# nannau/DoWnGAN

Measured on AMD Instinct MI355X. Metric: train-step samples/sec (G+D+GP), higher is better.
Workload: dtype bf16

## Files before the change

### downgan_amd/_lib.py

```python
from __future__ import annotations

import ctypes as C
import os

_HERE = os.path.dirname(os.path.abspath(__file__))
LIB_PATH = os.environ.get("DG_LIB_OVERRIDE") or os.path.join(_HERE, "csrc", "libdowngan_hip.so")

DG_F32, DG_BF16 = 0, 1
STATUS = {0: "DG_OK", -1: "DG_ERR_BAD_SHAPE", -2: "DG_ERR_BAD_DTYPE", -3: "DG_ERR_BAD_ARG", -4: "DG_ERR_LAUNCH"}


class Epilogue(C.Structure):
    _fields_ = [("bias", C.c_void_p), ("has_act", C.c_int), ("act_slope", C.c_float),
                ("r1", C.c_void_p), ("ldr1", C.c_int64), ("s1", C.c_float),
                ("r2", C.c_void_p), ("ldr2", C.c_int64), ("s2", C.c_float),
                ("mask", C.c_void_p), ("ldmask", C.c_int64), ("mask_slope", C.c_float),
                ("accumulate", C.c_int), ("mask_bits", C.c_void_p), ("out_bits", C.c_void_p),
                ("mask_c0", C.c_int), ("mask_last", C.c_int), ("out_q", C.c_void_p), ("out_qs", C.c_void_p), ("ldqs", C.c_int64),
                ("out_u", C.c_void_p), ("out_ue", C.c_void_p), ("skip_y", C.c_int), ("out_amax", C.c_void_p)]


class ConvGeom(C.Structure):
    _fields_ = [("dtype", C.c_int), ("N", C.c_int), ("H", C.c_int), ("W", C.c_int),
                ("Cin", C.c_int), ("Cout", C.c_int), ("stride", C.c_int), ("cin_real", C.c_int), ("pixel_shuffle", C.c_int),
# ... 110 lines not shown

class TemporalSpec(C.Structure):
    _fields_ = [("speed_u", C.c_int), ("speed_v", C.c_int), ("nthr", C.c_int), ("ndur", C.c_int), ("nlag", C.c_int),
                ("nbins", C.c_int), ("below", C.c_int * TEMPORAL_MAX_THR), ("lag", C.c_int * TEMPORAL_MAX_LAGS),
                ("scale", C.c_float * EOF_MAX_C), ("offset", C.c_float * EOF_MAX_C),
                ("thr", (C.c_float * TEMPORAL_MAX_THR) * HIST_MAX_OUT), ("lo", (C.c_float * TEMPORAL_MAX_LAGS) * HIST_MAX_OUT),
                ("inv_w", (C.c_float * TEMPORAL_MAX_LAGS) * HIST_MAX_OUT)]


MINMAX_PARTS = 256
_vp, _i, _i64, _f = C.c_void_p, C.c_int, C.c_int64, C.c_float
_PROTOS = {
    "dg_conv3x3_fwd": [C.POINTER(ConvGeom), C.POINTER(Epilogue), _vp, _vp, _vp, _vp],
    "dg_conv3x3_dgrad": [C.POINTER(ConvGeom), C.POINTER(Epilogue), _vp, _vp, _vp, _vp],
    "dg_conv3x3_wgrad": [C.POINTER(ConvGeom), _vp, _vp, _vp, _vp, _vp],
    "dg_conv3x3_wgrad_dense": [_vp, _i, _vp, _vp, _vp, _vp, _vp],
    "dg_conv3x3_wgrad_f8": [C.POINTER(ConvGeom), _vp, _vp, _vp, _vp, _vp, _vp],
    "dg_exp_from_amax": [_vp, _i, _i, _vp, _vp],
    "dg_conv3x3_wgrad_dense_f8": [C.POINTER(ConvGeom), _i, _vp, _vp, _vp, _vp, _vp, _vp],
    "dg_gather_gemm": [C.POINTER(GGDesc), C.POINTER(Epilogue), _vp, _vp, _vp, _vp],
    "dg_conv3x3_plan": [C.POINTER(ConvGeom), _i, C.POINTER(GGDesc)],
    "dg_last_conv_kernels": [],
    "dg_last_wgrad_kernel": [],
    "dg_conv3x3_dgrad_launches": [C.POINTER(ConvGeom)],
    "dg_conv3x3_dgrad_stream_eligible": [C.POINTER(ConvGeom), C.POINTER(Epilogue)],
    "dg_set_s2_dgrad_stream": [C.c_int],
    "dg_colsum": [_i, _vp, _i64, _i64, _i64, _i64, _i, _vp, _vp],
    "dg_colsum_multi": [_i, _vp, _i64, _i64, _i, _i, _vp, _vp],
    "dg_repack_conv_weights": [_i, _i, _vp, _vp, _i, _i, _vp],
    "dg_repack_dense_dgrad": [_i, _vp, _i, _i, _vp, _vp],
    "dg_wgrad_unswap": [_vp, _vp, _i, _i, _vp],
    "dg_linear_fwd": [_i, _vp, _i64, _vp, _i64, _vp, _i, _i, _i, _i64, _vp],
    "dg_linear_dx": [_i, _i, _vp, _i, _vp, _i64, _vp, _i64, _vp, _i64, _f, _i, _i, _i64, _vp],
    "dg_linear_dw": [_i, _vp, _i, _vp, _i64, _vp, _i64, _i, _i, _i64, _vp],
    "dg_linear_dw_wide": [_i, _vp, _i, _vp, _i64, _vp, _i64, _i, _i, _i64, _i, _vp],
    "dg_bias_act": [_i, _vp, _i, _vp, _vp, _i, _i, _i, _i, _f, _vp, _i, _f, _vp],
    "dg_mask_mul": [_i, _vp, _i64, _vp, _i64, _i64, _i, _f, _vp],
    "dg_axpby": [_i, _vp, _i64, _vp, _i64, _f, _vp, _i64, _f, _i64, _i, _vp],
    "dg_gp_interp": [_i, _vp, _vp, _vp, _vp, _i, _i64, _vp],
    "dg_gp_interp_c2": [_i, _vp, _vp, _i64, _vp, _vp, _vp, _vp, _i, _i64, _vp],
    "dg_scale_rows_c2": [_i, _vp, _i64, _vp, _vp, _i, _i64, _vp],
    "dg_sumsq_rows": [_i, _vp, _i, _i64, _vp, _vp],
    "dg_gp_finish": [_vp, _i, _i, _f, _f, _vp, _vp, _vp],
    "dg_scale_rows": [_i, _vp, _vp, _vp, _i, _i64, _vp],
    "dg_l1": [_i, _vp, _i64, _vp, _i64, _i64, _i, _vp, _vp, _i64, _f, _vp, _i64, _vp],
    "dg_sqdiff": [_i, _vp, _i64, _vp, _i64, _i64, _i, _vp, _vp],
    "dg_sum_strided": [_vp, _i, _i, _f, _vp, _vp],
    "dg_fill_col": [_vp, _i, _i, _i, _f, _vp],
    "dg_adam": [_vp, _vp, _vp, _vp, _vp, _i64, _f, _f, _f, _f, _i, _f, _vp],
    "dg_nchw_to_nhwc": [_i, _vp, _vp, _i, _i, _i, _i, _i, _vp],
    "dg_nhwc_to_nchw": [_i, _vp, _i64, _vp, _i, _i, _i, _i, _vp],
    "dg_cast": [_i, _vp, _vp, _i64, _vp],
    "dg_minmax_partial": [_i, _vp, _i64, _i64, _i, _vp, _vp],
    "dg_minmax_finish": [_vp, _i, _vp, _vp],
    "dg_normalise_planar": [_i, _vp, _i, _i, _i, _i64, _i, _vp, _vp, _vp],
    "dg_ssim_level": [_vp, _vp, _i, _i, _i, C.POINTER(SsimParams), _vp, _vp],
    "dg_avgpool2": [_vp, _vp, _i, _i, _i, _vp],
    "dg_msssim_finish": [_vp, _i, _i, C.POINTER(MsssimCombine), _vp, _vp],
    "dg_div_vort_sums": [_i, _vp, _i64, _vp, _i64, _i, _i, _i, _vp, _vp],
    "dg_gather_samples": [_i, _vp, _i64, _i, _vp, _i, _vp, _i, _vp],
    "dg_quant_mxfp8": [_i, _vp, _i64, _i64, _i, _vp, _i64, _vp, _i64, _vp],
    "dg_block_exp_max": [_vp, _i64, _i64, _i, _i, _vp, _vp, _vp],
    "dg_block_exp_max_batch": [C.POINTER(ExpBatch), _i, _vp, _vp],
    "dg_quant_uniform": [_i, _vp, _i64, _i64, _i, _vp, _vp, _i64, _vp],
    "dg_conv3x3_fwd_f8": [C.POINTER(ConvGeom), C.POINTER(Epilogue), C.POINTER(F8Operands), _vp, _vp],
    "dg_conv3x3_dgrad_f8": [C.POINTER(ConvGeom), C.POINTER(Epilogue), C.POINTER(F8Operands), _vp, _vp],
# ... 120 lines not shown
```

### downgan_amd/csrc/elementwise.hip

```cpp
#include <cstdlib>
#include "dg_internal.h"
#include <type_traits>

#include <math.h>

static inline unsigned ew_blocks(long long nthreads) {
  long long b = (nthreads + 255) / 256;
  if (b > 256 * 16) b = 256 * 16;
  if (b < 1) b = 1;
  return (unsigned)b;
}

template <typename T> __device__ __forceinline__ void ldc(const T* p, float* v) {
  ld4(p, v);
  if constexpr (DT<T>::EPC == 8) ld4(p + 4, v + 4);
}
template <typename T> __device__ __forceinline__ void stc(T* p, const float* v) {
  st4(p, v);
  if constexpr (DT<T>::EPC == 8) st4(p + 4, v + 4);
}

template <typename T>
__global__ void mask_mul_kernel(T* u, long long ldu, const T* y, long long ldy, long long rows, int cchunks, float slope) {
  constexpr int EPC = DT<T>::EPC;
// ... 394 lines not shown
}
extern "C" int dg_bias_act(int out_dtype, const float* in, int ldi, const float* bias, void* out, int ldo, int rows, int C,
                           int has_act, float slope, const void* mask, int ldmask, float mask_slope, void* stream) {
  if (!in || !out || rows <= 0 || C <= 0) return DG_ERR_BAD_SHAPE;
  hipStream_t st = reinterpret_cast<hipStream_t>(stream);
  const unsigned nb = ew_blocks((long long)rows * C);
  if (out_dtype == DG_F32) hipLaunchKernelGGL(bias_act_kernel<float>, dim3(nb), dim3(256), 0, st, in, ldi, bias, (float*)out, ldo, rows, C, has_act, slope, (const float*)mask, ldmask, mask_slope);
  else if (out_dtype == DG_BF16) hipLaunchKernelGGL(bias_act_kernel<bf16_t>, dim3(nb), dim3(256), 0, st, in, ldi, bias, (bf16_t*)out, ldo, rows, C, has_act, slope, (const bf16_t*)mask, ldmask, mask_slope);
  else return DG_ERR_BAD_DTYPE;
  return dg_check_launch();
}

__global__ void sum_strided_kernel(const float* in, int n, int stride, float scale, float* out) {
  float s = 0.f;
  for (int i = threadIdx.x; i < n; i += 64) s += in[(long long)i * stride];
  s = wave_sum(s);
  if (threadIdx.x == 0) out[0] = s * scale;
}
extern "C" int dg_sum_strided(const float* in, int n, int stride, float scale, float* out, void* stream) {
  if (!in || !out || n <= 0) return DG_ERR_BAD_ARG;
  hipLaunchKernelGGL(sum_strided_kernel, dim3(1), dim3(64), 0, reinterpret_cast<hipStream_t>(stream), in, n, stride, scale, out);
  return dg_check_launch();
}

__global__ void fill_col_kernel(float* buf, int rows, int ld, int col, float value) {
  for (int r = blockIdx.x * blockDim.x + threadIdx.x; r < rows; r += gridDim.x * blockDim.x) buf[(long long)r * ld + col] = value;
}
extern "C" int dg_fill_col(float* buf, int rows, int ld, int col, float value, void* stream) {
  if (!buf || rows <= 0) return DG_ERR_BAD_ARG;
  hipLaunchKernelGGL(fill_col_kernel, dim3(ew_blocks(rows)), dim3(256), 0, reinterpret_cast<hipStream_t>(stream), buf, rows, ld, col, value);
  return dg_check_launch();
}

__global__ void adam_kernel(float* p, const float* g, float* m, float* v, bf16_t* shadow, long long n4, float step_size,
                            float beta1, float beta2, float eps, float inv_sqrt_bc2, float gscale) {
  for (long long i = (long long)blockIdx.x * blockDim.x + threadIdx.x; i < n4; i += (long long)gridDim.x * blockDim.x) {
    float4 pv = reinterpret_cast<float4*>(p)[i];
    const float4 gv = reinterpret_cast<const float4*>(g)[i];
    float4 mv = reinterpret_cast<float4*>(m)[i];
    float4 vv = reinterpret_cast<float4*>(v)[i];
    float pa[4] = {pv.x, pv.y, pv.z, pv.w}, ga[4] = {gv.x, gv.y, gv.z, gv.w};
    float ma[4] = {mv.x, mv.y, mv.z, mv.w}, va[4] = {vv.x, vv.y, vv.z, vv.w};
#pragma unroll
    for (int e = 0; e < 4; ++e) {
      const float gg = ga[e] * gscale;
      ma[e] = beta1 * ma[e] + (1.f - beta1) * gg;
      va[e] = beta2 * va[e] + (1.f - beta2) * gg * gg;
      const float denom = sqrtf(va[e]) * inv_sqrt_bc2 + eps;
      pa[e] -= step_size * (ma[e] / denom);
    }
    reinterpret_cast<float4*>(p)[i] = make_float4(pa[0], pa[1], pa[2], pa[3]);
    reinterpret_cast<float4*>(m)[i] = make_float4(ma[0], ma[1], ma[2], ma[3]);
    reinterpret_cast<float4*>(v)[i] = make_float4(va[0], va[1], va[2], va[3]);
    if (shadow) st4(shadow + 4 * i, pa);
  }
}
extern "C" int dg_adam(float* p, const float* g, float* m, float* v, void* shadow_bf16, int64_t n, float lr, float beta1,
                       float beta2, float eps, int step, float grad_scale, void* stream) {
  if (!p || !g || !m || !v || n <= 0 || n % 4 || step < 1) return DG_ERR_BAD_ARG;
  const double bc1 = 1.0 - pow((double)beta1, step), bc2 = 1.0 - pow((double)beta2, step);
  hipLaunchKernelGGL(adam_kernel, dim3(ew_blocks(n / 4)), dim3(256), 0, reinterpret_cast<hipStream_t>(stream), p, g, m, v,
                     (bf16_t*)shadow_bf16, (long long)(n / 4), (float)(lr / bc1), beta1, beta2, eps, (float)(1.0 / sqrt(bc2)), grad_scale);
  return dg_check_launch();
}

template <typename T>
__global__ void nchw_to_nhwc_kernel(const float* src, T* dst, int N, int C, int H, int W, int Cpad) {
  const long long npix = (long long)N * H * W, hw = (long long)H * W;
  const long long total = npix * Cpad;
  for (long long i = (long long)blockIdx.x * blockDim.x + threadIdx.x; i < total; i += (long long)gridDim.x * blockDim.x) {
    const int c = (int)(i / npix); const long long pix = i % npix;
    const long long n = pix / hw, r = pix % hw;
    const float v = c < C ? src[(n * C + c) * hw + r] : 0.f;
    st_elem(dst + pix * Cpad + c, v);
  }
}
extern "C" int dg_nchw_to_nhwc(int dtype, const float* src, void* dst, int N, int C, int H, int W, int Cpad, void* stream) {
  if (!src || !dst || N <= 0 || C <= 0 || H <= 0 || W <= 0 || Cpad < C) return DG_ERR_BAD_SHAPE;
  hipStream_t st = reinterpret_cast<hipStream_t>(stream);
  const unsigned nb = ew_blocks((long long)N * H * W * Cpad);
  if (dtype == DG_F32) hipLaunchKernelGGL(nchw_to_nhwc_kernel<float>, dim3(nb), dim3(256), 0, st, src, (float*)dst, N, C, H, W, Cpad);
  else if (dtype == DG_BF16) hipLaunchKernelGGL(nchw_to_nhwc_kernel<bf16_t>, dim3(nb), dim3(256), 0, st, src, (bf16_t*)dst, N, C, H, W, Cpad);
  else return DG_ERR_BAD_DTYPE;
// ... 129 lines not shown
```

### downgan_amd/csrc/linear.hip

```cpp
#include "dg_internal.h"
#include <stdlib.h>

template <typename T> struct MmaL;
template <> struct MmaL<bf16_t> {
  static __device__ __forceinline__ void run(const uint4& a, const uint4& b, f32x4_t& c) {
    c = __builtin_amdgcn_mfma_f32_16x16x32_bf16(__builtin_bit_cast(bf16x8_t, a), __builtin_bit_cast(bf16x8_t, b), c, 0, 0, 0);
  }
};
template <> struct MmaL<float> {
  static __device__ __forceinline__ void run(const uint4& a, const uint4& b, f32x4_t& c) {
    c = __builtin_amdgcn_mfma_f32_16x16x4f32(__uint_as_float(a.x), __uint_as_float(b.x), c, 0, 0, 0);
    c = __builtin_amdgcn_mfma_f32_16x16x4f32(__uint_as_float(a.y), __uint_as_float(b.y), c, 0, 0, 0);
    c = __builtin_amdgcn_mfma_f32_16x16x4f32(__uint_as_float(a.z), __uint_as_float(b.z), c, 0, 0, 0);
    c = __builtin_amdgcn_mfma_f32_16x16x4f32(__uint_as_float(a.w), __uint_as_float(b.w), c, 0, 0, 0);
  }
};

typedef __attribute__((ext_vector_type(2))) float dg_f32x2_t;
template <typename T> struct LdX4;
typedef __attribute__((ext_vector_type(2))) unsigned int dg_u32x2_t;
template <> struct LdX4<float> {
  typedef dg_u32x4_t raw;
  static __device__ __forceinline__ raw load(const float* row, unsigned voff) {
    return __builtin_amdgcn_raw_buffer_load_b128(__builtin_amdgcn_make_buffer_rsrc((void*)row, 0, -1, 0x00020000), voff, 0, 0);
// ... 224 lines not shown
        acc[4 * q + e][0] = __builtin_elementwise_fma(d2, wa, acc[4 * q + e][0]);
        acc[4 * q + e][1] = __builtin_elementwise_fma(d2, wb, acc[4 * q + e][1]);
      }
  };
  auto wrow = [&](int o) { return LdX4<T>::load(w + (long long)(o < O ? o : O - 1) * ldw, voff); };
  constexpr int PD = 6;
  typename LdX4<T>::raw wq[PD];
#pragma unroll
  for (int u = 0; u < PD; ++u) wq[u] = wrow(u);
  read_row(d[0], 0);
  for (int o = 0; o < O; o += PD) {
#pragma unroll
    for (int u = 0; u < PD; ++u) {
      read_row(d[(u + 1) & 1], o + u + 1 < O ? o + u + 1 : O);
      landed(d[u & 1]);
      row_fma(wq[u], d[u & 1]);
      wq[u] = wrow(o + u + PD);
    }
  }
#pragma unroll
  for (int b = 0; b < BG; ++b) {
    if (b0 + b >= B) break;
    float v[4] = {acc[b][0][0], acc[b][0][1], acc[b][1][0], acc[b][1][1]};
    if (mask) {
      float mv[4];
      ld4(mask + (long long)(b0 + b) * ldmask + k, mv);
#pragma unroll
      for (int e = 0; e < 4; ++e) v[e] *= leaky_grad(mv[e], slope);
    }
    st4(dx + (long long)(b0 + b) * lddx + k, v);
  }
}

extern "C" int dg_linear_dx(int dtype, int out_dtype, const float* dy, int ldo, const void* w, int64_t ldw, void* dx,
                            int64_t lddx, const void* mask, int64_t ldmask, float mask_slope, int B, int O, int64_t K,
                            void* stream) {
  if (!dy || !w || !dx) return DG_ERR_BAD_ARG;
  if (B <= 0 || O <= 0 || O > 128 || K <= 0 || K % 8 || ldw % 8 || lddx % 8) return DG_ERR_BAD_SHAPE;
  if (mask && ldmask % 8) return DG_ERR_BAD_SHAPE;
  hipStream_t st = reinterpret_cast<hipStream_t>(stream);
  if (K >= 4096 && (long long)K * 4 < (1ll << 32) && B >= 16) {
    dim3 gridw((unsigned)((K / 4 + 255) / 256), (unsigned)((B + 31) / 32));
    if (dtype == DG_F32 && out_dtype == DG_F32) {
      hipLaunchKernelGGL((lin_dx_wide_kernel<float, float>), gridw, dim3(256), 0, st, dy, ldo, (const float*)w, (long long)ldw, (float*)dx,
                         (long long)lddx, (const float*)mask, (long long)ldmask, mask_slope, B, O, (long long)K);
      return dg_check_launch();
    }
    if (dtype == DG_BF16 && out_dtype == DG_BF16) {
      hipLaunchKernelGGL((lin_dx_wide_kernel<bf16_t, bf16_t>), gridw, dim3(256), 0, st, dy, ldo, (const bf16_t*)w, (long long)ldw, (bf16_t*)dx,
                         (long long)lddx, (const bf16_t*)mask, (long long)ldmask, mask_slope, B, O, (long long)K);
      return dg_check_launch();
    }
  }
  constexpr int BG = 16;
  const int epc = dtype == DG_F32 ? 4 : 8;
  dim3 grid((unsigned)((K / epc + 255) / 256), (unsigned)((B + BG - 1) / BG));
  if (dtype == DG_F32 && out_dtype == DG_F32)
    hipLaunchKernelGGL((lin_dx_kernel<float, float, BG>), grid, dim3(256), 0, st, dy, ldo, (const float*)w, ldw,
                       (float*)dx, lddx, (const float*)mask, ldmask, mask_slope, B, O, K);
  else if (dtype == DG_BF16 && out_dtype == DG_BF16)
    hipLaunchKernelGGL((lin_dx_kernel<bf16_t, bf16_t, BG>), grid, dim3(256), 0, st, dy, ldo, (const bf16_t*)w, ldw,
                       (bf16_t*)dx, lddx, (const bf16_t*)mask, ldmask, mask_slope, B, O, K);
  else if (dtype == DG_BF16 && out_dtype == DG_F32)
    hipLaunchKernelGGL((lin_dx_kernel<bf16_t, float, BG>), grid, dim3(256), 0, st, dy, ldo, (const bf16_t*)w, ldw,
                       (float*)dx, lddx, (const bf16_t*)mask, ldmask, mask_slope, B, O, K);
  else
    return DG_ERR_BAD_DTYPE;
  return dg_check_launch();
}

template <typename T, int OT>
__global__ __launch_bounds__(256) void lin_dw_kernel(const float* __restrict__ dy, int ldo, const T* __restrict__ x,
                                                     long long ldx, float* dw, long long lddw, int B, int O,
// ... 137 lines not shown
```

### downgan_amd/engine.py

```python
from __future__ import annotations

import dataclasses
import math
import os

import torch

from . import layout
from .ops import Conv

G_SLOPE = 0.01
C_SLOPE = 0.2
RES_SCALE = 0.2
FC_HID = 100
FC_HID_P = 112
FC_HID_LD = 128
FC_OUT_P = 16


@dataclasses.dataclass
class HyperParams:
    gp_lambda: float = 10.0
    critic_iterations: int = 5
    batch_size: int = 32
    gamma: float = 0.01
    content_lambda: float = 5.0
    lr: float = 0.00025
    beta1: float = 0.9
    beta2: float = 0.99
    eps: float = 1e-8


class ParamStore:

    def __init__(self, ops):
        self.ops = ops
        self.entries = {}
        self.size = 0
        self.conv_dgrad = {}
        self.after_refresh = []
        self._pending = None

    def add(self, name, shape):
        n = int(math.prod(shape))
        assert n % 4 == 0, (name, shape)
        self.entries[name] = (self.size, n, tuple(shape))
        self.size += n

    def finalize(self):
        o = self.ops
        self.p = o.zeros(self.size, dtype=torch.float32)
        self.g = o.zeros(self.size, dtype=torch.float32)
        self.m = o.zeros(self.size, dtype=torch.float32)
        self.v = o.zeros(self.size, dtype=torch.float32)
        self.shadow = self.p if o.tdtype == torch.float32 else o.zeros(self.size)
        self.dgrad_pack = {k: o.zeros(co * 9 * ci) for k, (co, ci) in self.conv_dgrad.items()}
        self.t = 0

    def defer(self, fn):
        self.sync()
        self._pending = fn

    def sync(self):
        fn, self._pending = self._pending, None
        if fn is not None:
            fn()

    def view(self, buf, name):
        if self._pending is not None:
            self.sync()
        off, n, shape = self.entries[name]
        return buf[off:off + n].view(shape)

    def master(self, name):
        return self.view(self.p, name)

    def grad(self, name):
        return self.view(self.g, name)

    def w(self, name):
        if self._pending is not None:
            self.sync()
        off, n, _ = self.entries[name]
        return self.shadow[off:off + n]

    def w2d(self, name):
        return self.view(self.shadow, name)

    def wd(self, name):
        if self._pending is not None:
            self.sync()
        return self.dgrad_pack[name]

    def refresh(self, shadow_done=False):
        o = self.ops
        if o.tdtype != torch.float32 and not shadow_done:
            o.cast(self.p, self.shadow)
        for name, (co, ci) in self.conv_dgrad.items():
            o.repack(self.master(name).reshape(-1), self.dgrad_pack[name], co, ci, 1)
        for fn in self.after_refresh:
            fn()

    def zero_grad(self, skip=None):
        self.sync()
        if skip is None:
            self.g.zero_()
        else:
            off, n, _ = self.entries[skip]
            self.g[:off].zero_()
            self.g[off + n:].zero_()

    def adam_step(self, hp: HyperParams, grad_scale=1.0):
        self.t += 1
        o = self.ops
        o.adam(self.p, self.g, self.m, self.v, None if o.tdtype == torch.float32 else self.shadow,
               hp.lr, hp.beta1, hp.beta2, hp.eps, self.t, grad_scale)
        self.refresh(shadow_done=True)

    def load_host(self, packed: dict):
        self.sync()
        host = torch.zeros(self.size, dtype=torch.float32)
        for name, t in packed.items():
            off, n, shape = self.entries[name]
            assert tuple(t.shape) == shape, (name, t.shape, shape)
            host[off:off + n] = t.reshape(-1)
        self.p.copy_(host)
        self.refresh()

    def export_state(self):
        self.sync()
        return self.p, self.m, self.v, self.t

    def import_state(self, state):
        p, m, v, t = state
        assert p.numel() == self.size, (p.numel(), self.size)
        self.sync()
        self.p.copy_(p); self.m.copy_(m); self.v.copy_(v)
        self.t = int(t)
        self.refresh()

    def to_host(self, buf=None):
        self.sync()
        h = (self.p if buf is None else buf).detach().cpu()
        return {name: h[off:off + n].view(shape).clone() for name, (off, n, shape) in self.entries.items()}


class NativeCritic:

    STRIDES = (1, 2, 1, 2, 1, 2, 1, 2)

    def __init__(self, ops, coarse_dim, fine_dim, nc, batch, stacked=False):
        assert fine_dim % 16 == 0, "critic.py:95 needs fine_dim divisible by 16"
        self.ops, self.B = ops, batch
        self.cd, self.fine, self.nc = coarse_dim, fine_dim, nc
        cd = coarse_dim
        self.c_real = [nc, cd, cd, 2 * cd, 2 * cd, 4 * cd, 4 * cd, 8 * cd, 8 * cd]
        self.c_pad = [layout.pad16(c) for c in self.c_real]
        self.convs = []
        h = fine_dim
        for l, st in enumerate(self.STRIDES):
            self.convs.append(Conv(batch, h, h, self.c_pad[l], self.c_pad[l + 1], st, False,
                                   cin_real=(nc if l == 0 and nc <= 2 else 0), net="C",
                                   cin_alg=self.c_real[l], cout_alg=self.c_real[l + 1]))
            h //= st
        self.hf = h
        self.fc_k = h * h * self.c_pad[8]
        P = self.P = ParamStore(ops)
        for l, cv in enumerate(self.convs):
            P.add(f"features.{2 * l}.weight", (cv.Cout, 9, cv.Cin))
            P.conv_dgrad[f"features.{2 * l}.weight"] = (cv.Cout, cv.Cin)
        P.add("features.0.bias", (self.c_pad[1],))
        P.add("classifier.0.weight", (FC_HID_P, self.fc_k))
        P.add("classifier.0.bias", (FC_HID_LD,))
        P.add("classifier.2.weight", (FC_OUT_P, FC_HID_LD))
        P.add("classifier.2.bias", (FC_OUT_P,))
        P.finalize()
        o = ops
        use_bits = os.environ.get("DG_NO_MASK_BITS") is None and all(c >= 128 and c % 64 == 0 for c in self.c_pad[1:])
        self.f8 = bool(getattr(o, "f8", False))
        self.stacked = bool(stacked) and use_bits and not self.f8 and 3 * batch <= 128 and os.environ.get("DG_NO_FC1_FUSED") is None
        self.stack_from = (int(stacked) - 1 if (stacked is not True and int(stacked) > 1) else 0) if self.stacked else 0
        cap = 3 * batch if self.stacked else batch
        self.cap = cap
        full = lambda cv: (cap,) + tuple(o.out_shape(cv))[1:]
        self._acts_all = [o.zeros(*full(cv)) for cv in self.convs[:7]] + [None]
        self._us_all = [o.zeros(*full(cv)) for cv in self.convs]
        self._bits_all = [o.zeros(*o.bits_shape(full(cv)), dtype=torch.int16) for cv in self.convs] if use_bits else None
        self.acts = [a[:batch] if a is not None else o.zeros(*o.out_shape(self.convs[7])) for a in self._acts_all]
        self.us = [u[:batch] for u in self._us_all]
        self.act_bits = [b[:batch] for b in self._bits_all] if use_bits else None
        self._h1pre_all = o.zeros(cap, FC_HID_LD, dtype=torch.float32)
        self._h1_all = o.zeros(cap, FC_HID_LD)
        self._outpre_all = o.zeros(cap, FC_OUT_P, dtype=torch.float32)
        self._out_all = o.zeros(cap, FC_OUT_P, dtype=torch.float32)
        self._dout_all = o.zeros(cap, FC_OUT_P, dtype=torch.float32)
        self.uh1 = o.zeros(batch, FC_HID_LD, dtype=torch.float32)
        self._cv_cache = {}
        self._tan = self._th1pre = self._th1 = self._ones = None
        self.fc1_fused = 3 * batch <= 128 and os.environ.get("DG_NO_FC1_FUSED") is None
        if self.fc1_fused:
            self._y7_all = o.zeros(4 * batch, *self.acts[7].shape[1:])
            self._uh1_all = o.zeros(3 * batch, FC_HID_LD, dtype=torch.float32)
            self.acts[7] = self._y7_all[3 * batch:]
            if self.stacked:
                self._acts_all[7] = self._y7_all[:3 * batch]
        qbuf = lambda t: (o.zeros(*t.shape, dtype=torch.uint8), o.zeros(*t.shape[:-1], t.shape[-1] // 32, dtype=torch.uint8))
        self.actq = [None] * 8
        self.usq = [None] * 8
        self.wq_f, self.wq_d = [None] * 8, [None] * 8
# ... 331 lines not shown
                for p in range(3):
                    r = slice(p * B, (p + 1) * B)
                    o.conv_dgrad(cv1[l], self._us_all[l][r], P.wd(name), self._us_all[l - 1][r], mask_bits=self._bits_all[l - 1][r], mask_slope=C_SLOPE)
            elif l > 0:
                o.conv_dgrad(cv3[l], self._us_all[l], P.wd(name), self._us_all[l - 1], mask_bits=self._bits_all[l - 1], mask_slope=C_SLOPE)
            else:
                o.conv_dgrad(cv1[0], self._us_all[0][2 * B:], P.wd(name), dx)


class NativeGenerator:

    def __init__(self, ops, filters, channels, batch, coarse_side, n_predictands=2, num_res_blocks=16, num_upsample=3):
        assert filters % 16 == 0, "native path needs filters to be a multiple of 16"
        self.ops, self.B, self.S = ops, batch, coarse_side
        self.F, self.cin, self.npred = filters, channels, n_predictands
        self.cin_p, self.np_p = layout.pad16(channels), layout.pad16(n_predictands)
        self.nrb, self.nup = num_res_blocks, num_upsample
        F_, S, B = filters, coarse_side, batch
        self.cv_conv1 = Conv(B, S, S, self.cin_p, F_, cin_real=(channels if channels <= 2 else 0), cin_alg=channels)
        self.cv_b = [Conv(B, S, S, k * F_, F_, net="G") for k in range(1, 6)]
        self.cv_conv2 = Conv(B, S, S, F_, F_, net="G")
        self.cv_up = [Conv(B, S << u, S << u, F_, 4 * F_, 1, True, net="T") for u in range(num_upsample)]
        hs = S << num_upsample
        self.cv_c30 = Conv(B, hs, hs, F_, F_, net="T")
        self.cv_c32 = Conv(B, hs, hs, F_, self.np_p, cout_alg=n_predictands)
        self.cv_c32_bwd = Conv(B, hs, hs, self.np_p, F_, cin_real=n_predictands, cin_alg=n_predictands) if n_predictands <= 2 else None
        P = self.P = ParamStore(ops)
        for name, cv, _, _, dgrad in self._conv_layers():
            P.add(name + ".weight", (cv.Cout, 9, cv.Cin))
            P.add(name + ".bias", (cv.Cout,))
            if dgrad:
                P.conv_dgrad[name + ".weight"] = (cv.Cout, cv.Cin)
        P.finalize()
        o = ops
        self.ndrb = 3 * num_res_blocks
        self.out1 = o.zeros(B, S, S, F_)
        self.trunk = o.zeros(B, S, S, F_)
        self.ups = [o.zeros(B, S << (u + 1), S << (u + 1), F_) for u in range(num_upsample)]
        self.c30 = o.zeros(B, hs, hs, F_)
        self.fake = o.zeros(B, hs, hs, self.np_p)
        self._ring = [o.zeros(B, S, S, 5 * F_) for _ in range(4)]
        self._saved = None
        self._bwd = None
        self.f8 = bool(getattr(o, "f8_generator", False)) and all(o.f8_eligible(cv, "fwd") for cv in self.cv_b)
        self._qring = [(o.zeros(B, S, S, 5 * F_, dtype=torch.uint8), o.zeros(B, S, S, 5 * F_ // 32, dtype=torch.uint8)) for _ in range(4)] if self.f8 else None
        self.f8_tail = self.f8 and all(o.f8_eligible(cv, "fwd") for cv in self.cv_up + [self.cv_c30])
        self._tq = None
        self._w_c32_bwd = o.zeros(F_ * 9 * self.np_p) if self.cv_c32_bwd is not None else None
        self._dw_c32_tmp = None
        if self.cv_c32_bwd is not None:
            P.after_refresh.append(lambda: o.repack(P.master("conv3.2.weight").reshape(-1), self._w_c32_bwd, self.np_p, F_, 2))
        self._wq = {}
        self._vq = None
        self._qlast = None
        self.cv_v = [Conv(B, S, S, F_, (5 - j) * F_, net="G") for j in range(5)]
        self._vsize = [(5 - j) * F_ * 9 * F_ for j in range(5)]
        self._vpack = [o.zeros(sum(self._vsize)) for _ in range(self.ndrb)]
        self.f8_bwd = self.f8 and bool(getattr(o, "f8_gbwd", False)) and all(o.f8_eligible(cv, "dgrad") for cv in self.cv_v)
        self.f8_wg = (self.f8_bwd and bool(getattr(o, "f8_wgrad", False)) and bool(getattr(o, "f8_gwgrad", False)) and F_ == 128 and S % 64 == 0)
        self._slab_u = self._us_u = self._ex = self._eu = self._ex_new = self._eu_new = None
        self._u_ok = False
        self._u_live = False
        P.after_refresh.append(self._rebuild_vpacks)
        if self.f8:
            P.after_refresh.append(self._requantise_weights)

# ... 562 lines not shown
```

### downgan_amd/ops.py

```python
from __future__ import annotations

import ctypes as C
import dataclasses

import os
import torch

from . import _lib
from ._lib import ConvGeom, Epilogue, check

TORCH_DTYPE = {"f32": torch.float32, "bf16": torch.bfloat16}
DG_DTYPE = {"f32": _lib.DG_F32, "bf16": _lib.DG_BF16}


@dataclasses.dataclass(frozen=True)
class Conv:
    N: int
    H: int
    W: int
    Cin: int
    Cout: int
    stride: int = 1
    pixel_shuffle: bool = False
    cin_real: int = 0
# ... 93 lines not shown
        assert 1 <= len(bufs) <= _lib.FINITE_MAX
        f = _lib.FiniteBufs(nbuf=len(bufs))
        for i, (name, t) in enumerate(bufs):
            assert t.is_cuda and t.is_contiguous() and t.dtype in (torch.float32, torch.bfloat16), (name, t.dtype)
            f.ptr[i], f.n[i], f.dtype[i] = t.data_ptr(), t.numel(), (_lib.DG_F32 if t.dtype == torch.float32 else _lib.DG_BF16)
        if self._finite_counts is None:
            self._finite_counts = torch.zeros(_lib.FINITE_MAX, dtype=torch.int32, device=self.device)
        check(self.lib.dg_count_nonfinite(C.byref(f), _ptr(self._finite_counts), self._stream()), "dg_count_nonfinite")
        counts = self._finite_counts.cpu().tolist()
        return {name: int(counts[i]) for i, (name, _) in enumerate(bufs)}

    def _stream(self):
        if torch.cuda.current_device() != self._dev_index:
            torch.cuda.set_device(self.device)
        return C.c_void_p(torch.cuda.current_stream(self.device).cuda_stream)

    per_layer = False

    def _timed(self, tag, flops, fn, nbytes=0.0, net="", geom=""):
        if self.prof is None:
            return fn()
        s, e = torch.cuda.Event(enable_timing=True), torch.cuda.Event(enable_timing=True)
        s.record()
        rc = fn()
        e.record()
        if self.per_layer and geom:
            tag = f"{tag}:{geom}"
        if net:
            tag = f"{tag}:{net}"
        if tag.startswith(("conv_fwd", "conv_dgrad")):
            tag = f"{tag}:k{self.lib.dg_last_conv_kernels()}"
        self.prof.append((tag, flops, nbytes, s, e))
        return rc

    @staticmethod
    def _geom_tag(cv):
        return f"{cv.Cin}>{cv.Cout}@{cv.H}" + ("s2" if cv.stride == 2 else "") + ("ps" if cv.pixel_shuffle else "")

    @staticmethod
    def conv_flops(cv):
        return 2.0 * 9 * (cv.cin_alg or cv.Cin) * (cv.cout_alg or cv.Cout) * cv.Ho * cv.Wo * cv.N

    def conv_bytes(self, cv, ep=None):
        es = 2 if self.dtype == "bf16" else 4
        out = cv.N * cv.Ho * cv.Wo * cv.Cout
        extra = 0 if ep is None else sum(1 for k in ("r1", "r2") if ep.get(k) is not None) + int(bool(ep.get("accumulate")))
        if ep is not None and ep.get("mask") is not None:
            extra += 1.0 - float(ep.get("mask_c0", 0)) / cv.Cin if "mask_c0" in ep else 1
        return float(es * (cv.N * cv.H * cv.W * cv.Cin + out * (1 + extra) + 9 * cv.Cin * cv.Cout))

    def _act(self, t):
        assert t.dtype == self.tdtype and t.is_cuda, (t.dtype, t.device)
        return t

    def _geom(self, cv: Conv, ldx, ldy):
        return ConvGeom(dtype=self.dg, N=cv.N, H=cv.H, W=cv.W, Cin=cv.Cin, Cout=cv.Cout, stride=cv.stride,
                        cin_real=cv.cin_real, pixel_shuffle=int(cv.pixel_shuffle), ldx=ldx, ldy=ldy)

    @staticmethod
    def bits_shape(shape):
        N, H, W, Cc = shape
        assert Cc % 64 == 0 and Cc >= 128, Cc
        return (N, H, W, Cc // 64, 4)

    def _epilogue(self, out, bias=None, act=None, r1=None, s1=1.0, r2=None, s2=1.0, mask=None, mask_slope=1.0,
                  accumulate=False, mask_bits=None, out_bits=None, mask_c0=0, mask_last=False, out_q=None, out_u=None, skip_y=False,
# ... 235 lines not shown
    def colsum(self, dy, db):
        assert db.dtype == torch.float32
        dg = _lib.DG_F32 if dy.dtype == torch.float32 else self.dg
        if dy.dim() == 2:
            rows, ld, Cc = dy.shape[0], dy.stride(0), dy.shape[1]
        else:
            ld, rows = pix_layout(dy)
            Cc = dy.shape[-1]
        assert db.numel() >= Cc
        check(self.lib.dg_colsum(dg, _ptr(dy), rows, ld, 1, ld, Cc, _ptr(db), self._stream()), "dg_colsum")

    def colsum_multi(self, dy, dbs):
        self._act(dy)
        n, Cc = len(dbs), dy.shape[-1]
        assert Cc % n == 0 and all(d.dtype == torch.float32 and d.numel() >= Cc // n for d in dbs)
        ld, rows = pix_layout(dy)
        pb = (C.c_void_p * n)(*[t.data_ptr() for t in dbs])
        check(self._timed("ew_colsum", 0.0, lambda: self.lib.dg_colsum_multi(self.dg, _ptr(dy), rows, ld, Cc, n, pb, self._stream()),
                          float(dy.numel() * dy.element_size()), "G"), "dg_colsum_multi")

    def colsum_ps(self, dy, db):
        self._act(dy)
        ld, _ = pix_layout(dy)
        n, h2, w2, f = dy.shape
        for i in range(2):
            for j in range(2):
                sub = dy[:, i::2, j::2, :]
                check(self.lib.dg_colsum(self.dg, _ptr(sub), n * (h2 // 2), 2 * w2 * ld, w2 // 2, 2 * ld, f,
                                         _ptr(db[(2 * i + j) * f:]), self._stream()), "dg_colsum")

    def repack(self, master, dst, cout, cin, kind):
        assert master.dtype == torch.float32 and master.numel() == cout * 9 * cin
        assert dst.dtype == self.tdtype and dst.numel() == cout * 9 * cin
        check(self.lib.dg_repack_conv_weights(self.dg, kind, _ptr(master), _ptr(dst), cout, cin, self._stream()), "dg_repack_conv_weights")

    def repack_dense(self, masters, dst, F_):
        n = len(masters)
        for k, m in enumerate(masters):
            assert m.dtype == torch.float32 and m.is_contiguous() and m.numel() == F_ * 9 * (k + 1) * F_
        assert dst.dtype == self.tdtype and dst.is_contiguous() and dst.numel() == 9 * F_ * F_ * n * (n + 1) // 2
        pm = (C.c_void_p * n)(*[m.data_ptr() for m in masters])
        check(self.lib.dg_repack_dense_dgrad(self.dg, pm, n, F_, _ptr(dst), self._stream()), "dg_repack_dense_dgrad")

    def wgrad_unswap(self, tmp, dw, cout, cin):
        assert tmp.dtype == torch.float32 and dw.dtype == torch.float32 and tmp.numel() == dw.numel() == cout * 9 * cin
        check(self.lib.dg_wgrad_unswap(_ptr(tmp), _ptr(dw), cout, cin, self._stream()), "dg_wgrad_unswap")

    def linear_fwd(self, x, w, y, o_real=0, net=""):
        self._act(x); self._act(w)
        B, K = x.shape
        O = w.shape[0]
        assert w.shape[1] == K and y.dtype == torch.float32 and y.shape[0] == B and y.shape[1] >= O
        es = x.element_size()
        check(self._timed("lin_fwd", 2.0 * B * (o_real or O) * K, lambda: self.lib.dg_linear_fwd(
            self.dg, _ptr(x), x.stride(0), _ptr(w), w.stride(0), _ptr(y), y.stride(0), B, O, K, self._stream()),
            float(es * (B * K + O * K)), net), "dg_linear_fwd")

    def linear_dx(self, dy, w, dx, mask=None, mask_slope=1.0, o_real=0, net=""):
        self._act(w)
        B, K = dx.shape
        O = w.shape[0]
        assert dy.dtype == torch.float32 and dy.shape[0] == B and dy.shape[1] >= O and w.shape[1] == K
        out_dg = _lib.DG_F32 if dx.dtype == torch.float32 else self.dg
        if mask is not None:
            self._act(mask)
            assert mask.shape == dx.shape
        es = w.element_size()
# ... 541 lines not shown
```

### include/downgan_hip.h

```cpp
#ifndef DOWNGAN_HIP_H
#define DOWNGAN_HIP_H

#include <stddef.h>
#include <stdint.h>

#ifdef __cplusplus
extern "C" {
#endif

#define DG_F32 0
#define DG_BF16 1

typedef enum dg_status {
  DG_OK = 0,
  DG_ERR_BAD_SHAPE = -1,
  DG_ERR_BAD_DTYPE = -2,
  DG_ERR_BAD_ARG = -3,
  DG_ERR_LAUNCH = -4
} dg_status;

typedef struct dg_epilogue {
  const float* bias;
  int has_act;
  float act_slope;
// ... 59 lines not shown
                              float* const* dw, void* stream);

int dg_colsum(int dtype, const void* dy, int64_t rows_outer, int64_t ld_outer, int64_t rows_inner,
              int64_t ld, int C, float* db, void* stream);

int dg_colsum_multi(int dtype, const void* dy, int64_t rows, int64_t ld, int C, int nseg, float* const* db, void* stream);

int dg_gather_gemm(const dg_gg_desc* d, const dg_epilogue* ep, const void* x, const void* w, void* y,
                   void* stream);

int dg_last_conv_kernels(void);

int dg_last_wgrad_kernel(void);

int dg_conv3x3_plan(const dg_conv_geom* g, int kind, dg_gg_desc* out);

int dg_conv3x3_dgrad_launches(const dg_conv_geom* g);

int dg_conv3x3_dgrad_stream_eligible(const dg_conv_geom* g, const dg_epilogue* ep);

int dg_set_s2_dgrad_stream(int on);

int dg_repack_conv_weights(int dtype, int kind, const float* master, void* dst, int CoutP, int CinP,
                           void* stream);
int dg_repack_dense_dgrad(int dtype, const float* const* masters, int nconv, int F, void* dst, void* stream);
int dg_wgrad_unswap(const float* tmp, float* dw, int CoutP, int CinP, void* stream);


int dg_linear_fwd(int dtype, const void* x, int64_t ldx, const void* w, int64_t ldw, float* y,
                  int ldy, int B, int O, int64_t K, void* stream);
int dg_linear_dx(int dtype, int out_dtype, const float* dy, int ldo, const void* w, int64_t ldw,
                 void* dx, int64_t lddx, const void* mask, int64_t ldmask, float mask_slope, int B,
                 int O, int64_t K, void* stream);
int dg_linear_dw(int dtype, const float* dy, int ldo, const void* x, int64_t ldx, float* dw,
                 int64_t lddw, int B, int O, int64_t K, void* stream);
int dg_linear_dw_wide(int dtype, const float* dy, int ldo, const void* x, int64_t ldx, float* dw,
                      int64_t lddw, int B, int O, int64_t K, int accumulate, void* stream);


int dg_bias_act(int out_dtype, const float* in, int ldi, const float* bias, void* out, int ldo,
                int rows, int C, int has_act, float slope, const void* mask, int ldmask,
                float mask_slope, void* stream);
int dg_mask_mul(int dtype, void* u, int64_t ldu, const void* y, int64_t ldy, int64_t rows, int C,
                float slope, void* stream);
int dg_axpby(int dtype, void* out, int64_t ldo, const void* x, int64_t ldx, float a, const void* y,
             int64_t ldy, float b, int64_t rows, int C, void* stream);
int dg_gp_interp(int dtype, const void* real, const void* fake, const float* alpha, void* xhat,
                 int B, int64_t per_img, void* stream);
int dg_gp_interp_c2(int dtype, const void* real, const void* fake, int64_t ld, const float* alpha,
                    void* xhat_c, void* real_c, void* fake_c, int B, int64_t pix_per_img, void* stream);
int dg_scale_rows_c2(int dtype, const void* g, int64_t ld, const float* coef, void* out_c, int B,
                     int64_t pix_per_img, void* stream);
int dg_sumsq_rows(int dtype, const void* g, int B, int64_t per_img, float* ss, void* stream);
int dg_gp_finish(const float* ss, int B, int B_global, float gp_lambda, float weight, float* coef,
                 float* scalars, void* stream);
int dg_scale_rows(int dtype, const void* g, const float* coef, void* out, int B, int64_t per_img,
                  void* stream);
int dg_l1(int dtype, const void* a, int64_t lda, const void* b, int64_t ldb, int64_t rows, int C,
          float* acc, void* grad, int64_t ldg, float grad_scale, const void* addend, int64_t ldadd,
          void* stream);
int dg_sqdiff(int dtype, const void* a, int64_t lda, const void* b, int64_t ldb, int64_t rows, int C,
              float* acc, void* stream);
int dg_sum_strided(const float* in, int n, int stride, float scale, float* out, void* stream);
int dg_fill_col(float* buf, int rows, int ld, int col, float value, void* stream);

int dg_adam(float* p, const float* g, float* m, float* v, void* shadow_bf16, int64_t n, float lr,
// ... 271 lines not shown
```

Baseline: 73.61.

## Add MFMA bf16 linear dgrad kernel and skip Adam on frozen padded rows

Adds an MFMA-based dx kernel for the bf16 linear layer. It is used by default when K is at least 65536 and O is at most 128. The float32 dy is split into three bf16 pieces to keep near-fp32 accuracy, and weights are transposed through LDS with ds_read_tr16. The Adam step now skips padded rows of the critic's first FC weight, which are marked frozen, so it no longer spends bandwidth on dead parameters. Adam arithmetic is also rewritten with fmaf, and profiling hooks are added around zero_grad, Adam and repack.

```diff
diff --git a/downgan_amd/_lib.py b/downgan_amd/_lib.py
--- a/downgan_amd/_lib.py
+++ b/downgan_amd/_lib.py
@@ -166,6 +166,9 @@
     "dg_wgrad_unswap": [_vp, _vp, _i, _i, _vp],
     "dg_linear_fwd": [_i, _vp, _i64, _vp, _i64, _vp, _i, _i, _i, _i64, _vp],
     "dg_linear_dx": [_i, _i, _vp, _i, _vp, _i64, _vp, _i64, _vp, _i64, _f, _i, _i, _i64, _vp],
+    "dg_set_linear_mfma": [C.c_int],
+    "dg_linear_dx_mfma_eligible": [_i, _i, _vp, _i64, _vp, _i64, _vp, _i64, _i, _i, _i64],
+    "dg_last_linear_kernel": [],
     "dg_linear_dw": [_i, _vp, _i, _vp, _i64, _vp, _i64, _i, _i, _i64, _vp],
     "dg_linear_dw_wide": [_i, _vp, _i, _vp, _i64, _vp, _i64, _i, _i, _i64, _i, _vp],
     "dg_bias_act": [_i, _vp, _i, _vp, _vp, _i, _i, _i, _i, _f, _vp, _i, _f, _vp],
diff --git a/downgan_amd/csrc/elementwise.hip b/downgan_amd/csrc/elementwise.hip
--- a/downgan_amd/csrc/elementwise.hip
+++ b/downgan_amd/csrc/elementwise.hip
@@ -450,6 +450,14 @@
   return dg_check_launch();
 }
 
+__device__ __forceinline__ void adam_elem(float& p, float g, float& m, float& v, float step_size, float beta1, float beta2,
+                                          float eps, float inv_sqrt_bc2, float gscale) {
+  const float gg = g * gscale;
+  m = fmaf(beta1, m, (1.f - beta1) * gg);
+  v = fmaf(beta2, v, (1.f - beta2) * gg * gg);
+  const float denom = fmaf(sqrtf(v), inv_sqrt_bc2, eps);
+  p = fmaf(-step_size, m / denom, p);
+}
 __global__ void adam_kernel(float* p, const float* g, float* m, float* v, bf16_t* shadow, long long n4, float step_size,
                             float beta1, float beta2, float eps, float inv_sqrt_bc2, float gscale) {
   for (long long i = (long long)blockIdx.x * blockDim.x + threadIdx.x; i < n4; i += (long long)gridDim.x * blockDim.x) {
@@ -460,13 +468,7 @@
     float pa[4] = {pv.x, pv.y, pv.z, pv.w}, ga[4] = {gv.x, gv.y, gv.z, gv.w};
     float ma[4] = {mv.x, mv.y, mv.z, mv.w}, va[4] = {vv.x, vv.y, vv.z, vv.w};
 #pragma unroll
-    for (int e = 0; e < 4; ++e) {
-      const float gg = ga[e] * gscale;
-      ma[e] = beta1 * ma[e] + (1.f - beta1) * gg;
-      va[e] = beta2 * va[e] + (1.f - beta2) * gg * gg;
-      const float denom = sqrtf(va[e]) * inv_sqrt_bc2 + eps;
-      pa[e] -= step_size * (ma[e] / denom);
-    }
+    for (int e = 0; e < 4; ++e) adam_elem(pa[e], ga[e], ma[e], va[e], step_size, beta1, beta2, eps, inv_sqrt_bc2, gscale);
     reinterpret_cast<float4*>(p)[i] = make_float4(pa[0], pa[1], pa[2], pa[3]);
     reinterpret_cast<float4*>(m)[i] = make_float4(ma[0], ma[1], ma[2], ma[3]);
     reinterpret_cast<float4*>(v)[i] = make_float4(va[0], va[1], va[2], va[3]);
diff --git a/downgan_amd/csrc/linear.hip b/downgan_amd/csrc/linear.hip
--- a/downgan_amd/csrc/linear.hip
+++ b/downgan_amd/csrc/linear.hip
@@ -280,6 +280,147 @@
   }
 }
 
+constexpr int DXM_TK = 128;
+constexpr int DXM_PITCH = 2 * DXM_TK + 64;
+constexpr int DXM_OLD = DXM_TK + 4;
+constexpr int DXM_NW = 8, DXM_NM = 2;
+typedef __attribute__((address_space(3))) s16x4_t* lds_s16x4_lin_ptr;
+
+__global__ __launch_bounds__(256, 2) void lin_dx_mfma_kernel(const float* __restrict__ dy, int ldo, const bf16_t* __restrict__ w,
+                                                             long long ldw, bf16_t* dx, long long lddx, const bf16_t* mask,
+                                                             long long ldmask, float slope, int B, int O, long long K,
+                                                             long long ntiles) {
+  __shared__ __attribute__((aligned(16))) unsigned char sw[128 * DXM_PITCH];
+  __shared__ __attribute__((aligned(16))) float so[32 * DXM_OLD];
+  const int tid = threadIdx.x, lane = tid & 63, wave = tid >> 6;
+  const int l15 = lane & 15, g = lane >> 4, q = l15 >> 2, pp = l15 & 3;
+  const int b0 = blockIdx.y * 32;
+  const int nnt = B - b0 > 16 ? 2 : 1, nkk = (O + 31) / 32;
+  for (int i = tid; i < 128 * DXM_PITCH / 16; i += 256) reinterpret_cast<uint4*>(sw)[i] = make_uint4(0u, 0u, 0u, 0u);
+
+  typedef __attribute__((ext_vector_type(8))) unsigned short u16x8_t;
+  bf16x8_t dyf[2][4][3];
+#pragma unroll
+  for (int nt = 0; nt < 2; ++nt)
+#pragma unroll
+    for (int kk = 0; kk < 4; ++kk) {
+      u16x8_t t0, t1, t2;
+      const int b = b0 + 16 * nt + l15;
+#pragma unroll
+      for (int j = 0; j < 8; ++j) {
+        const int o = 32 * kk + 8 * g + j;
+        const float v = (b < B && o < O) ? dy[(long long)b * ldo + o] : 0.f;
+        const unsigned hb = __float_as_uint(v) & 0xffff0000u;
+        const float r1 = v - __uint_as_float(hb);
+        const unsigned mb = __float_as_uint(r1) & 0xffff0000u;
+        const float r2 = r1 - __uint_as_float(mb);
+        t0[j] = (unsigned short)(hb >> 16); t1[j] = (unsigned short)(mb >> 16); t2[j] = (unsigned short)(__float_as_uint(r2) >> 16);
+      }
+      dyf[nt][kk][0] = __builtin_bit_cast(bf16x8_t, t0);
+      dyf[nt][kk][1] = __builtin_bit_cast(bf16x8_t, t1);
+      dyf[nt][kk][2] = __builtin_bit_cast(bf16x8_t, t2);
+    }
+
+  const int crow = tid >> 4, ccol = (tid & 15) * 8;
+  uint4 wr[DXM_NW], mr[DXM_NM], mc[DXM_NM];
+  auto fetch = [&](long long t) {
+    const long long k = t * DXM_TK + ccol;
+    const bool kin = k < K;
+#pragma unroll
+    for (int i = 0; i < DXM_NW; ++i) {
+      const int o = crow + 16 * i;
+      wr[i] = make_uint4(0u, 0u, 0u, 0u);
+      if (kin && o < O) wr[i] = *reinterpret_cast<const uint4*>(w + (long long)o * ldw + k);
+    }
+#pragma unroll
+    for (int i = 0; i < DXM_NM; ++i) {
+      const int b = b0 + crow + 16 * i;
+      mr[i] = make_uint4(0u, 0u, 0u, 0u);
+      if (mask && kin && b < B) mr[i] = *reinterpret_cast<const uint4*>(mask + (long long)b * ldmask + k);
+    }
+  };
+  const unsigned char* const tr0 = sw + (8 * g + q) * DXM_PITCH + 8 * pp;
+
+  long long t = blockIdx.x;
+  if (t < ntiles) fetch(t);
+  __syncthreads();
+  for (; t < ntiles; t += gridDim.x) {
+#pragma unroll
+    for (int i = 0; i < DXM_NW; ++i) {
+      const int o = crow + 16 * i;
+      if (o < O) *reinterpret_cast<uint4*>(sw + o * DXM_PITCH + 2 * ccol) = wr[i];
+    }
+#pragma unroll
+    for (int i = 0; i < DXM_NM; ++i) mc[i] = mr[i];
+    __syncthreads();
+    if (t + gridDim.x < ntiles) fetch(t + gridDim.x);
+    f32x4_t acc[2][2];
+#pragma unroll
+    for (int a = 0; a < 2; ++a) acc[a][0] = acc[a][1] = f32x4_t{0.f, 0.f, 0.f, 0.f};
+#pragma unroll
+    for (int kk = 0; kk < 4; ++kk) {
+      if (kk >= nkk) break;
+#pragma unroll
+      for (int a = 0; a < 2; ++a) {
+        const unsigned char* pa = tr0 + kk * 32 * DXM_PITCH + (2 * wave + a) * 32;
+        const s16x4_t lo = __builtin_amdgcn_ds_read_tr16_b64_v4i16((lds_s16x4_lin_ptr)(pa));
+        const s16x4_t hi = __builtin_amdgcn_ds_read_tr16_b64_v4i16((lds_s16x4_lin_ptr)(pa + 4 * DXM_PITCH));
+        typedef __attribute__((ext_vector_type(8))) short s16x8_t;
+        const s16x8_t v = {lo[0], lo[1], lo[2], lo[3], hi[0], hi[1], hi[2], hi[3]};
+        const bf16x8_t fa = __builtin_bit_cast(bf16x8_t, v);
+#pragma unroll
+        for (int nt = 0; nt < 2; ++nt) {
+          if (nt >= nnt) break;
+#pragma unroll
+          for (int s = 2; s >= 0; --s) acc[a][nt] = __builtin_amdgcn_mfma_f32_16x16x32_bf16(fa, dyf[nt][kk][s], acc[a][nt], 0, 0, 0);
+        }
+      }
+    }
+#pragma unroll
+    for (int a = 0; a < 2; ++a)
+#pragma unroll
+      for (int nt = 0; nt < 2; ++nt)
+        *reinterpret_cast<f32x4_t*>(so + (16 * nt + l15) * DXM_OLD + (2 * wave + a) * 16 + 4 * g) = acc[a][nt];
+    __syncthreads();
+    const long long k = t * DXM_TK + ccol;
+#pragma unroll
+    for (int i = 0; i < DXM_NM; ++i) {
+      const int br = crow + 16 * i;
+      if (k >= K || b0 + br >= B) continue;
+      const float4 v0 = *reinterpret_cast<const float4*>(so + br * DXM_OLD + ccol);
+      const float4 v1 = *reinterpret_cast<const float4*>(so + br * DXM_OLD + ccol + 4);
+      float v[8] = {v0.x, v0.y, v0.z, v0.w, v1.x, v1.y, v1.z, v1.w};
+      if (mask) {
+        const unsigned mw[4] = {mc[i].x, mc[i].y, mc[i].z, mc[i].w};
+#pragma unroll
+        for (int e = 0; e < 4; ++e) {
+          v[2 * e] *= leaky_grad(__uint_as_float(mw[e] << 16), slope);
+          v[2 * e + 1] *= leaky_grad(__uint_as_float(mw[e] & 0xffff0000u), slope);
+        }
+      }
+      *reinterpret_cast<uint4*>(dx + (long long)(b0 + br) * lddx + k) =
+          make_uint4(pack_bf16x2(v[0], v[1]), pack_bf16x2(v[2], v[3]), pack_bf16x2(v[4], v[5]), pack_bf16x2(v[6], v[7]));
+    }
+  }
+}
+
+static std::atomic<int> g_lin_mfma{1};
+static std::atomic<int> g_last_lin{0};
+extern "C" int dg_set_linear_mfma(int on) { return g_lin_mfma.exchange(on < 0 ? 0 : on, std::memory_order_relaxed); }
+extern "C" int dg_last_linear_kernel(void) { return g_last_lin.load(std::memory_order_relaxed); }
+static int lin_dx_mfma_can(int dtype, int out_dtype, const void* w, int64_t ldw, const void* dx, int64_t lddx, const void* mask,
+                           int64_t ldmask, int B, int O, int64_t K) {
+  if (dtype != DG_BF16 || out_dtype != DG_BF16) return 0;
+  if (B < 1 || O <= 0 || O > 128 || K < 4096 || K % 8 || ldw % 8 || lddx % 8 || ldw < K || lddx < K) return 0;
+  if (((uintptr_t)w | (uintptr_t)dx) & 15) return 0;
+  if (mask && (ldmask % 8 || ldmask < K || ((uintptr_t)mask & 15))) return 0;
+  return 1;
+}
+extern "C" int dg_linear_dx_mfma_eligible(int dtype, int out_dtype, const void* w, int64_t ldw, const void* dx, int64_t lddx,
+                                          const void* mask, int64_t ldmask, int B, int O, int64_t K) {
+  return K >= 65536 && lin_dx_mfma_can(dtype, out_dtype, w, ldw, dx, lddx, mask, ldmask, B, O, K);
+}
+
 extern "C" int dg_linear_dx(int dtype, int out_dtype, const float* dy, int ldo, const void* w, int64_t ldw, void* dx,
                             int64_t lddx, const void* mask, int64_t ldmask, float mask_slope, int B, int O, int64_t K,
                             void* stream) {
@@ -287,6 +428,17 @@
   if (B <= 0 || O <= 0 || O > 128 || K <= 0 || K % 8 || ldw % 8 || lddx % 8) return DG_ERR_BAD_SHAPE;
   if (mask && ldmask % 8) return DG_ERR_BAD_SHAPE;
   hipStream_t st = reinterpret_cast<hipStream_t>(stream);
+  const int mfma_mode = g_lin_mfma.load(std::memory_order_relaxed);
+  if (mfma_mode >= 2 ? lin_dx_mfma_can(dtype, out_dtype, w, ldw, dx, lddx, mask, ldmask, B, O, K)
+                     : mfma_mode == 1 && dg_linear_dx_mfma_eligible(dtype, out_dtype, w, ldw, dx, lddx, mask, ldmask, B, O, K)) {
+    const long long ntiles = ((long long)K + DXM_TK - 1) / DXM_TK;
+    dim3 gridm((unsigned)(ntiles < 512 ? ntiles : 512), (unsigned)((B + 31) / 32));
+    hipLaunchKernelGGL(lin_dx_mfma_kernel, gridm, dim3(256), 0, st, dy, ldo, (const bf16_t*)w, (long long)ldw, (bf16_t*)dx,
+                       (long long)lddx, (const bf16_t*)mask, (long long)ldmask, mask_slope, B, O, (long long)K, ntiles);
+    g_last_lin.store(3, std::memory_order_relaxed);
+    return dg_check_launch();
+  }
+  g_last_lin.store(K >= 4096 && (long long)K * 4 < (1ll << 32) && B >= 16 && dtype == out_dtype ? 2 : 1, std::memory_order_relaxed);
   if (K >= 4096 && (long long)K * 4 < (1ll << 32) && B >= 16) {
     dim3 gridw((unsigned)((K / 4 + 255) / 256), (unsigned)((B + 31) / 32));
     if (dtype == DG_F32 && out_dtype == DG_F32) {
diff --git a/downgan_amd/engine.py b/downgan_amd/engine.py
--- a/downgan_amd/engine.py
+++ b/downgan_amd/engine.py
@@ -40,6 +40,8 @@
         self.conv_dgrad = {}
         self.after_refresh = []
         self._pending = None
+        self.frozen = []
+        self.net = ""
 
     def add(self, name, shape):
         n = int(math.prod(shape))
@@ -101,20 +103,46 @@
         for fn in self.after_refresh:
             fn()
 
+    def _timed(self, tag, nbytes, fn):
+        timed = getattr(self.ops, "timed", None)
+        return fn() if timed is None else timed(tag, nbytes, fn)
+
     def zero_grad(self, skip=None):
         self.sync()
-        if skip is None:
-            self.g.zero_()
-        else:
-            off, n, _ = self.entries[skip]
-            self.g[:off].zero_()
-            self.g[off + n:].zero_()
+
+        def fill():
+            if skip is None:
+                self.g.zero_()
+            else:
+                off, n, _ = self.entries[skip]
+                self.g[:off].zero_()
+                self.g[off + n:].zero_()
+        self._timed("zero_grad", 4.0 * (self.size - (0 if skip is None else self.entries[skip][1])), fill)
+
+    def freeze_rows(self, name, r0):
+        off, n, shape = self.entries[name]
+        assert len(shape) == 2 and 0 < r0 <= shape[0]
+        if r0 < shape[0]:
+            self.frozen.append((off + r0 * shape[1], off + n))
+
+    def adam_ranges(self):
+        out, a = [], 0
+        for f0, f1 in sorted(self.frozen):
+            if f0 > a:
+                out.append((a, f0))
+            a = max(a, f1)
+        if a < self.size:
+            out.append((a, self.size))
+        return out
 
     def adam_step(self, hp: HyperParams, grad_scale=1.0):
         self.t += 1
         o = self.ops
-        o.adam(self.p, self.g, self.m, self.v, None if o.tdtype == torch.float32 else self.shadow,
-               hp.lr, hp.beta1, hp.beta2, hp.eps, self.t, grad_scale)
+        es = 28.0 if o.tdtype == torch.float32 else 30.0
+        for a, b in self.adam_ranges():
+            self._timed("adam_" + (self.net or "net"), es * (b - a), lambda: o.adam(
+                self.p[a:b], self.g[a:b], self.m[a:b], self.v[a:b], None if o.tdtype == torch.float32 else self.shadow[a:b],
+                hp.lr, hp.beta1, hp.beta2, hp.eps, self.t, grad_scale))
         self.refresh(shadow_done=True)
 
     def load_host(self, packed: dict):
@@ -175,6 +203,8 @@
         P.add("classifier.2.weight", (FC_OUT_P, FC_HID_LD))
         P.add("classifier.2.bias", (FC_OUT_P,))
         P.finalize()
+        P.net = "C"
+        P.freeze_rows("classifier.0.weight", FC_HID)
         o = ops
         use_bits = os.environ.get("DG_NO_MASK_BITS") is None and all(c >= 128 and c % 64 == 0 for c in self.c_pad[1:])
         self.f8 = bool(getattr(o, "f8", False))
@@ -572,6 +602,7 @@
             if dgrad:
                 P.conv_dgrad[name + ".weight"] = (cv.Cout, cv.Cin)
         P.finalize()
+        P.net = "G"
         o = ops
         self.ndrb = 3 * num_res_blocks
         self.out1 = o.zeros(B, S, S, F_)
diff --git a/downgan_amd/ops.py b/downgan_amd/ops.py
--- a/downgan_amd/ops.py
+++ b/downgan_amd/ops.py
@@ -149,6 +149,9 @@
             tag = f"{tag}:k{self.lib.dg_last_conv_kernels()}"
         self.prof.append((tag, flops, nbytes, s, e))
         return rc
+
+    def timed(self, tag, nbytes, fn):
+        return self._timed(tag, 0.0, fn, float(nbytes))
 
     @staticmethod
     def _geom_tag(cv):
@@ -450,7 +453,9 @@
     def repack(self, master, dst, cout, cin, kind):
         assert master.dtype == torch.float32 and master.numel() == cout * 9 * cin
         assert dst.dtype == self.tdtype and dst.numel() == cout * 9 * cin
-        check(self.lib.dg_repack_conv_weights(self.dg, kind, _ptr(master), _ptr(dst), cout, cin, self._stream()), "dg_repack_conv_weights")
+        check(self._timed("repack", 0.0, lambda: self.lib.dg_repack_conv_weights(
+            self.dg, kind, _ptr(master), _ptr(dst), cout, cin, self._stream()),
+            float((4 + dst.element_size()) * master.numel())), "dg_repack_conv_weights")
 
     def repack_dense(self, masters, dst, F_):
         n = len(masters)
diff --git a/include/downgan_hip.h b/include/downgan_hip.h
--- a/include/downgan_hip.h
+++ b/include/downgan_hip.h
@@ -115,6 +115,11 @@
 int dg_linear_dx(int dtype, int out_dtype, const float* dy, int ldo, const void* w, int64_t ldw,
                  void* dx, int64_t lddx, const void* mask, int64_t ldmask, float mask_slope, int B,
                  int O, int64_t K, void* stream);
+
+int dg_set_linear_mfma(int on);
+int dg_linear_dx_mfma_eligible(int dtype, int out_dtype, const void* w, int64_t ldw, const void* dx, int64_t lddx,
+                               const void* mask, int64_t ldmask, int B, int O, int64_t K);
+int dg_last_linear_kernel(void);
 int dg_linear_dw(int dtype, const float* dy, int ldo, const void* x, int64_t ldx, float* dw,
                  int64_t lddw, int B, int O, int64_t K, void* stream);
 int dg_linear_dw_wide(int dtype, const float* dy, int ldo, const void* x, int64_t ldx, float* dw,
```

Result: no change. 73.71 (median of 6 runs) (+0.1%).
